# sbi-dev/sbi

Hardware: AMD Instinct MI355X
Metric: NPE train (theta,x)-pairs/sec (higher is better)
Workload: dtype f32; 1 GPU; BASELINE configs[1]: NPE + NSF theta-dim 10, x-dim 10, 100000 simulations (90 000-row training split resident in HBM), batch 65536 per GPU, synthetic linear-Gaussian; step = shuffled batch gather (device sampler) + fused NPE training step (pack, loss fwd+bwd, grad all-reduce, clip+Adam); parallelism=dp1, rccl_ranks=1

## Files before the change

sbi_amd/csrc/nsf_train_kernel.h:

```cpp
#pragma once
#include <hip/hip_runtime.h>
#include <stdlib.h>
#include <string.h>
#include "nsf_device.h"
#include "nsf_plan_layout.h"

#define TR_NW 4
#define TR_ROWS 64
#define TR_MAXCH 4
#define TR_GRID_MAX 256
#define TR_SA 68
#define TR_SB 68
#define TR_SLOT(PT) (16 * (PT) + 1)
#define TR_LDK_FAST 50
#ifndef TR_LA
#define TR_LA 2
#endif
#ifndef TR_SPLINE_PRIO
#define TR_SPLINE_PRIO 0
#endif
#ifndef TR_H_SPLIT
#define TR_H_SPLIT 0
#endif
#ifndef TR_PSTASH
#define TR_PSTASH 1
#endif
#ifndef TR_NO_S0
#define TR_NO_S0 1
#endif

struct TrainPlan {
  int SA, SB, SS;
  int o_A0, o_A1, o_B, o_Bs, o_cnt;
  int o_xs;
  int o_wave, w_total;
  int w_zs, w_gys, w_gzs;
  int DCHB, PTW;
  int nch[2];
  int PLP;
  int grid, ntiles;
  int lds_floats;
  int overlay;
  float* grad_x;
};

constexpr int build_train_layout(const NsfPlan& pl, TrainPlan* tp) {
  if (pl.D > 15 || pl.H > 64 || pl.NB > 2 || (pl.NB < 1 && !pl.ctx_mlp)) return SBI_AMD_E_UNSUPPORTED;
  const int d_id_max = pl.shape[0].d_id > pl.shape[1].d_id ? pl.shape[0].d_id : pl.shape[1].d_id;
  if (d_id_max + pl.C + 1 > 32 || pl.C + 1 > 32) return SBI_AMD_E_UNSUPPORTED;
  tp->DCHB = 4 / pl.PT;
  if (tp->DCHB < 1) return SBI_AMD_E_UNSUPPORTED;
  if (tp->DCHB > 2) tp->DCHB = 2;
  tp->PTW = 16 * pl.PT;
  for (int par = 0; par < 2; ++par) {
    tp->nch[par] = (pl.shape[par].d_tr + tp->DCHB - 1) / tp->DCHB;
    if (tp->nch[par] > TR_MAXCH) return SBI_AMD_E_UNSUPPORTED;
  }
  tp->SA = TR_SA;
  tp->SB = TR_SB;
  {
    const int in0max = d_id_max + pl.C;
    const int nt0 = (in0max + 1 + 15) / 16, ntc = (pl.C + 1 + 15) / 16;
    int need = 16 * nt0 > d_id_max + 16 * ntc ? 16 * nt0 : d_id_max + 16 * ntc;
    tp->SS = (need + 3) / 4 * 4;
    if ((tp->SS / 4) % 2 == 0) tp->SS += 4;
  }
  int w = 0;
  tp->w_zs = w; w += 16 * pl.ZW;
  tp->w_gys = w; w += 16 * pl.ZW;
  tp->w_gzs = w; w += 16 * pl.ZW;
  tp->w_total = (w + 16 + 3) / 4 * 4;
  for (int ov = 0; ov < 2; ++ov) {
    const int fin_min = pl.shape[0].final_off < pl.shape[1].final_off ? pl.shape[0].final_off : pl.shape[1].final_off;
    int o = ov ? (pl.hidden_img_floats > pl.lds_w_train_floats - fin_min ? pl.hidden_img_floats
                                                                         : pl.lds_w_train_floats - fin_min)
               : pl.lds_w_train_floats;
    o = (o + 3) / 4 * 4;
    tp->overlay = ov;
    tp->o_A0 = o; o += TR_ROWS * tp->SA;
    tp->o_A1 = o; o += TR_ROWS * tp->SA;
    tp->o_B = o; o += TR_ROWS * tp->SB;
    tp->o_Bs = o; o += TR_ROWS * tp->SS;
    tp->o_cnt = o; o += 4;
    tp->o_xs = o; o += 64;
    tp->o_wave = o;
    tp->lds_floats = tp->o_wave + TR_NW * tp->w_total;
    if (4ll * tp->lds_floats <= NSF_LDS_LIMIT_BYTES) break;
  }
  if (4ll * tp->lds_floats > NSF_LDS_LIMIT_BYTES) return SBI_AMD_E_LDS;
  int pmax = pl.shape[0].n_params > pl.shape[1].n_params ? pl.shape[0].n_params : pl.shape[1].n_params;
  tp->PLP = (pmax + 1 + 3) / 4 * 4;
  tp->grad_x = nullptr;
  tp->ntiles = 0;
  tp->grid = 0;
  return 0;
}
static int build_train_plan(const NsfPlan& pl, int64_t n, TrainPlan* tp) {
  *tp = TrainPlan{};
  const int rc = build_train_layout(pl, tp);
  if (rc) return rc;
  tp->ntiles = (int)((n + TR_ROWS - 1) / TR_ROWS);
  tp->grid = tp->ntiles < TR_GRID_MAX ? tp->ntiles : TR_GRID_MAX;
  if (NSF_DBG_ABL(pl.ablate, 512) && tp->grid > 4) tp->grid = 4;
  return 0;
}

constexpr sbi_amd_nsf_config kNsfDefaultCfg = {10, 10, 50, 10, 5, 2, 3.0f, 1e-3f, 1e-3f, 1e-3f, 1e-3f};
constexpr NsfPlan nsf_make_static_plan() {
  NsfPlan p{};
  nsf_build_layout(&kNsfDefaultCfg, TR_NW, &p);
  return p;
}
constexpr NsfPlan kStaticPl = nsf_make_static_plan();
constexpr TrainPlan nsf_make_static_train() {
  TrainPlan t{};
  build_train_layout(kStaticPl, &t);
  return t;
}
constexpr TrainPlan kStaticTp = nsf_make_static_train();
static_assert(kStaticPl.n_params == 98025 && kStaticTp.overlay == 0 && kStaticTp.nch[0] == 3, "default NSF layout");

static bool plan_is_static_default(const NsfPlan& pl, const TrainPlan& tp) {
  NsfPlan a = pl;
  a.B = a.min_w = a.min_h = a.min_d = a.lu_eps = a.sqrt_h = a.inv_sqrt_h = 0.f;
  a.one_minus_kw = a.one_minus_kh = a.d_const = a.log_z = 0.f;
  a.ablate = 0;
  const NsfPlan b = kStaticPl;
  if (memcmp(&a, &b, sizeof(NsfPlan)) != 0) return false;
  TrainPlan c = tp;
  c.grid = c.ntiles = 0;
  c.grad_x = nullptr;
  const TrainPlan d = kStaticTp;
  return memcmp(&c, &d, sizeof(TrainPlan)) == 0 && NSF_DBG_ABL(pl.ablate, 0x40000) == 0;
}

__device__ __forceinline__ void stage_D(float* __restrict__ st, int SA, int row, const LaneId& id,
                                        const f4 (&v)[NSF_HT], bool relu) {
#pragma unroll
  for (int mt = 0; mt < NSF_HT; ++mt)
#pragma unroll
    for (int r = 0; r < 4; ++r) {
      float a = v[mt][r];
      st[row * SA + 16 * mt + 4 * r + id.g] = relu ? fmaxf(a, 0.f) : a;
    }
}

__device__ __forceinline__ int il_col(int c) { return 4 * (c & 15) + (c >> 4); }
__device__ __forceinline__ void stage_DB(float* __restrict__ st, int SB, int row, const LaneId& id,
                                         const f4 (&v)[NSF_HT], bool relu) {
  static_assert(NSF_HT == 4, "one float4 per register row");
#pragma unroll
  for (int r = 0; r < 4; ++r) {
    f4 w = {v[0][r], v[1][r], v[2][r], v[3][r]};
    if (relu) w = {fmaxf(w[0], 0.f), fmaxf(w[1], 0.f), fmaxf(w[2], 0.f), fmaxf(w[3], 0.f)};
    *(f4*)(st + row * SB + 4 * (4 * r + id.g)) = w;
  }
}

__device__ __forceinline__ constexpr int dw_krow(int s) { return 16 * (s >> 2) + (s & 3); }

template <int NT, int SA, int SB, bool IL = false>
__device__ __forceinline__ void dw_gemm(const float* __restrict__ Ast, const float* __restrict__ Bst,
                                        int acol0, int bcol0, const LaneId& id, f4 (&acc)[NT], int nt_on = NT,
                                        int abl = 0, f4* accb = nullptr) {
  if (abl & 1) return;
  const float ones_b = id.j == 0 ? 1.f : 0.f;
  constexpr int KS = TR_ROWS / 4, LA = NT >= 3 ? TR_LA : 2 * TR_LA;
  const float* ap = Ast + 4 * id.g * SA + acol0 + id.j;
  const float* bp = IL ? Bst + 4 * id.g * SB + 4 * id.j + (bcol0 >> 4) : Bst + 4 * id.g * SB + bcol0 + id.j;
  float a[LA + 1], b[LA + 1][NT];
  auto load_b = [&](int u, int s) {
    if (IL && NT == 4) {
      const f4 w = *(const f4*)(bp + dw_krow(s) * SB);
#pragma unroll
      for (int nt = 0; nt < NT; ++nt) b[u][nt] = w[nt];
    } else {
#pragma unroll
      for (int nt = 0; nt < NT; ++nt) b[u][nt] = bp[dw_krow(s) * SB + (IL ? nt : 16 * nt)];
    }
  };
#pragma unroll
  for (int u = 0; u < LA; ++u) {
    a[u] = ap[dw_krow(u) * SA];
    load_b(u, u);
  }
#pragma unroll
  for (int s = 0; s < KS; ++s) {
    if (s + LA < KS) {
      a[(s + LA) % (LA + 1)] = ap[dw_krow(s + LA) * SA];
      load_b((s + LA) % (LA + 1), s + LA);
    }
    __builtin_amdgcn_sched_barrier(0);
#pragma unroll
    for (int nt = 0; nt < NT; ++nt)
      if (NT == 1 || nt < nt_on) acc[nt] = MFMA16(a[s % (LA + 1)], b[s % (LA + 1)][nt], acc[nt]);
    if (accb) *accb = MFMA16(a[s % (LA + 1)], ones_b, *accb);
    __builtin_amdgcn_sched_barrier(0);
  }
}

template <int NT, int SA>
__device__ __forceinline__ void dw_gemm_rs(const float* __restrict__ Ast, const float* __restrict__ Bst, int SBr,
                                           int acol0, int bcol0, const LaneId& id, f4 (&acc)[NT], int nt_on = NT,
                                           int abl = 0) {
  if (abl & 1) return;
  constexpr int KS = TR_ROWS / 4, LA = NT >= 4 ? TR_LA : 2 * TR_LA;
  const float* ap = Ast + 4 * id.g * SA + acol0 + id.j;
  const float* bp = Bst + 4 * id.g * SBr + bcol0 + id.j;
  float a[LA + 1], b[LA + 1][NT];
#pragma unroll
  for (int u = 0; u < LA; ++u) {
    a[u] = ap[dw_krow(u) * SA];
#pragma unroll
    for (int nt = 0; nt < NT; ++nt) b[u][nt] = bp[dw_krow(u) * SBr + 16 * nt];
  }
#pragma unroll
  for (int s = 0; s < KS; ++s) {
    if (s + LA < KS) {
      a[(s + LA) % (LA + 1)] = ap[dw_krow(s + LA) * SA];
#pragma unroll
      for (int nt = 0; nt < NT; ++nt) b[(s + LA) % (LA + 1)][nt] = bp[dw_krow(s + LA) * SBr + 16 * nt];
    }
    __builtin_amdgcn_sched_barrier(0);
#pragma unroll
    for (int nt = 0; nt < NT; ++nt)
      if (NT == 1 || nt < nt_on) acc[nt] = MFMA16(a[s % (LA + 1)], b[s % (LA + 1)][nt], acc[nt]);
    __builtin_amdgcn_sched_barrier(0);
  }
}

#define MFMA4(a, b, c) __builtin_amdgcn_mfma_f32_4x4x1f32((a), (b), (c), 0, 0, 0)
constexpr int TR_THIN_C0 = 48;
static_assert(kStaticPl.H == TR_THIN_C0 + 2 && kStaticPl.KSH == 13 && kStaticPl.NB == 2,
              "thin remainder: the static layout's hidden width leaves 2 real features (+ bias column) in tile 3");

template <int SA, int SB>
__device__ __forceinline__ void dw_thin(const float* __restrict__ Ast, const float* __restrict__ Bst, const LaneId& id,
                                        f4& accM, f4& accN) {
  const int l = id.lane;
  const float* aM = Ast + TR_THIN_C0 + (l & 3);
  const float* aN = Ast + l;
  const float* bM = Bst + il_col(l);
  const float* bN = Bst + il_col(TR_THIN_C0 + (l & 3));
  constexpr int KS = TR_ROWS / 4;
  float v[2][4][4];
  auto load = [&](int u, int s) {
#pragma unroll
    for (int g = 0; g < 4; ++g) {
      const int r = dw_krow(s) + 4 * g;
      v[u][g][0] = aM[r * SA];
      v[u][g][1] = bM[r * SB];
      v[u][g][2] = aN[r * SA];
      v[u][g][3] = bN[r * SB];
    }
  };
  load(0, 0);
#pragma unroll
  for (int s = 0; s < KS; ++s) {
    if (s + 1 < KS) load((s + 1) & 1, s + 1);
    __builtin_amdgcn_sched_barrier(0);
#pragma unroll
    for (int g = 0; g < 4; ++g) {
      accM = MFMA4(v[s & 1][g][0], v[s & 1][g][1], accM);
      accN = MFMA4(v[s & 1][g][2], v[s & 1][g][3], accN);
    }
    __builtin_amdgcn_sched_barrier(0);
  }
}
template <bool THIN>
__device__ __forceinline__ void dw_hidden(const float* __restrict__ Ast, const float* __restrict__ Bst, int gw,
                                          const LaneId& id, f4 (&acc)[4], int abl) {
  if constexpr (THIN) {
    if (abl & 1) return;
    if (gw == TR_NW - 1) dw_thin<TR_SA, TR_SB>(Ast, Bst, id, acc[0], acc[1]);
    else dw_gemm<3, TR_SA, TR_SB, true>(Ast, Bst, 16 * gw, 0, id, *reinterpret_cast<f4(*)[3]>(&acc[0]));
  } else {
    dw_gemm<4, TR_SA, TR_SB, true>(Ast, Bst, 16 * gw, 0, id, acc, 4, abl, nullptr);
  }
}

__device__ __forceinline__ void load_D(const float* __restrict__ st, int SA, int row, const LaneId& id,
                                       f4 (&v)[NSF_HT]) {
#pragma unroll
  for (int mt = 0; mt < NSF_HT; ++mt)
#pragma unroll
    for (int r = 0; r < 4; ++r) v[mt][r] = st[row * SA + 16 * mt + 4 * r + id.g];
}

__device__ __forceinline__ void grad_wave_sync(int* cnt, int target, int lane) {
  __builtin_amdgcn_fence(__ATOMIC_RELEASE, "workgroup");
  if (lane == 0) __hip_atomic_fetch_add(cnt, 1, __ATOMIC_RELAXED, __HIP_MEMORY_SCOPE_WORKGROUP);
  while (__hip_atomic_load(cnt, __ATOMIC_RELAXED, __HIP_MEMORY_SCOPE_WORKGROUP) < target) __builtin_amdgcn_s_sleep(1);
  __builtin_amdgcn_fence(__ATOMIC_ACQUIRE, "workgroup");
}

template <int KS, int MT, int LDK>
__device__ __forceinline__ void gemm_T_breg_ldk(const float* __restrict__ lds, const LinDesc& L, const LaneId& id,
                                                const f4 (&gb)[NSF_HT], f4 (&acc)[MT]) {
  const int ldk = LDK ? LDK : L.ldk;
  const float* base[MT];
#pragma unroll
  for (int mt = 0; mt < MT; ++mt) {
    const int f = 16 * mt + id.iperm;
    base[mt] = lds + L.l_w + id.g * ldk + (f < L.in ? f : 0);
  }
  const int kstride = 4 * ldk;
  constexpr int NP = (KS + 1) / 2;
  float a[2][2][MT];
#pragma unroll
  for (int u = 0; u < 2; ++u)
#pragma unroll
    for (int mt = 0; mt < MT; ++mt) a[0][u][mt] = u < KS ? base[mt][u * kstride] : 0.f;
#pragma unroll
  for (int p = 0; p < NP; ++p) {
    if (p + 1 < NP) {
#pragma unroll
      for (int u = 0; u < 2; ++u)
#pragma unroll
        for (int mt = 0; mt < MT; ++mt)
          a[(p + 1) & 1][u][mt] = (2 * p + 2 + u < KS) ? base[mt][(2 * p + 2 + u) * kstride] : 0.f;
    }
    __builtin_amdgcn_sched_barrier(0);
#pragma unroll
    for (int u = 0; u < 2; ++u) {
      const int s = 2 * p + u;
      if (s < KS) {
        const float bv = gb[s >> 2][s & 3];
#pragma unroll
        for (int mt = 0; mt < MT; ++mt) acc[mt] = MFMA16(a[p & 1][u][mt], bv, acc[mt]);
      }
    }
// ... 254 lines not shown
      }
    }
  }
#pragma unroll
  for (int mt = 0; mt < NSF_HT; ++mt)
#pragma unroll
    for (int r = 0; r < 4; ++r) gh[mt][r] = (16 * mt + 4 * r + id.g < LF.in) ? gh[mt][r] : 0.f;
}
template <int PT>
__device__ __forceinline__ void wft_chunk(const float* __restrict__ lds, const LinDesc& LF, const NsfPlan& pl,
                                          const ShapeDesc& S, const LaneId& id, const float* __restrict__ Arow,
                                          int SA, int d0, f4 (&gh)[NSF_HT]) {
  if (LF.ldk == TR_LDK_FAST) wft_chunk_ldk<PT, TR_LDK_FAST>(lds, LF, pl, S, id, Arow, SA, d0, gh);
  else wft_chunk_ldk<PT, 0>(lds, LF, pl, S, id, Arow, SA, d0, gh);
}

__device__ __forceinline__ void write_tile(float* __restrict__ part, const LinDesc& L, int out0, int nt,
                                           const LaneId& id, const f4& acc) {
#pragma unroll
  for (int r = 0; r < 4; ++r) {
    const int out = out0 + 4 * id.g + r;
    const int in = 16 * nt + id.j;
    if (out < L.out) {
      if (in < L.in) part[L.g_w + out * L.in + in] = acc[r];
      else if (in == L.in) part[L.g_b + out] = acc[r];
    }
  }
}
__device__ __forceinline__ void write_thin(float* __restrict__ part, const LinDesc& L, const LaneId& id, const f4& accM,
                                           const f4& accN) {
  const int l = id.lane;
#pragma unroll
  for (int m = 0; m < 4; ++m) {
    const int outM = TR_THIN_C0 + m, inM = l;
    if (outM < L.out) {
      if (inM < L.in) part[L.g_w + outM * L.in + inM] = accM[m];
      else if (inM == L.in) part[L.g_b + outM] = accM[m];
    }
    const int outN = 4 * (l >> 2) + m, inN = TR_THIN_C0 + (l & 3);
    if (l < TR_THIN_C0 && outN < L.out) {
      if (inN < L.in) part[L.g_w + outN * L.in + inN] = accN[m];
      else if (inN == L.in) part[L.g_b + outN] = accN[m];
    }
  }
}
__device__ __forceinline__ void write_bias(float* __restrict__ part, const LinDesc& L, int out0, const LaneId& id,
                                           const f4& accb) {
  if (id.j != 0) return;
#pragma unroll
  for (int r = 0; r < 4; ++r) {
    const int out = out0 + 4 * id.g + r;
    if (out < L.out) part[L.g_b + out] = accb[r];
  }
}

constexpr LinDesc wo_lin(int i) { return kStaticPl.shape[0].lin[i]; }
#define WO_LANE_WORDS(L, row0, in)                                    \
  const bool wcol_ = (in) < (L).in;                                   \
  const int off = wcol_ ? (L).g_w + ((row0) + 4 * g) * (L).in + (in) : (L).g_b + (row0) + 4 * g; \
  const int stride = wcol_ ? (L).in : 1;
template <int LI, int GW, int NT>
__device__ __forceinline__ void wo_tiles(float* __restrict__ part, int j, int g, const f4* acc) {
  constexpr LinDesc L = wo_lin(LI);
  constexpr int rem = L.out - 16 * GW;
  static_assert(rem >= 16 || (rem > 0 && rem <= 4), "a partial m-tile's live rows sit in lane group 0");
  constexpr int RL = rem >= 16 ? 4 : rem;
#pragma unroll
  for (int nt = 0; nt < NT; ++nt) {
    if (16 * nt > L.in) continue;
    const int in = 16 * nt + j;
    WO_LANE_WORDS(L, 16 * GW, in)
    bool live = in <= L.in;
    if (rem < 16) live = live && g == 0;
    if (live) {
#pragma unroll
      for (int r = 0; r < RL; ++r) part[off + r * stride] = acc[nt][r];
    }
  }
}
template <int LI>
__device__ __forceinline__ void wo_thin(float* __restrict__ part, int l, const f4& accM, const f4& accN) {
  constexpr LinDesc L = wo_lin(LI);
  static_assert(L.out == TR_THIN_C0 + 2 && L.in == L.out, "thin strips: a 50 x 50 hidden layer");
  if (l <= L.in) {
    const bool w = l < L.in;
    const int off = w ? L.g_w + TR_THIN_C0 * L.in + l : L.g_b + TR_THIN_C0;
    const int stride = w ? L.in : 1;
#pragma unroll
    for (int m = 0; m < L.out - TR_THIN_C0; ++m) part[off + m * stride] = accM[m];
  }
  const int in = TR_THIN_C0 + (l & 3);
  if (l < TR_THIN_C0 && in <= L.in) {
    const bool w = in < L.in;
    const int row = 4 * (l >> 2);
    const int off = w ? L.g_w + row * L.in + in : L.g_b + row;
    const int stride = w ? L.in : 1;
#pragma unroll
    for (int m = 0; m < 4; ++m) part[off + m * stride] = accN[m];
  }
}
template <int DD, int PTI, int NT0, int NTN>
__device__ __forceinline__ void wo_final(float* __restrict__ part, int j, int g, const f4* acc) {
  constexpr LinDesc L = wo_lin(kStaticPl.shape[0].fin);
  constexpr int P = kStaticPl.P;
  constexpr int rem = P - 16 * PTI;
  static_assert(rem > 0, "parameter tile");
  constexpr int GF = rem / 4, RP = rem % 4;
#pragma unroll
  for (int i = 0; i < NTN; ++i) {
    if (16 * (NT0 + i) > L.in) continue;
    const int in = 16 * (NT0 + i) + j;
    WO_LANE_WORDS(L, DD * P + 16 * PTI, in)
    const bool live = in <= L.in;
    if (live && g <= GF) {
#pragma unroll
      for (int r = 0; r < RP; ++r) part[off + r * stride] = acc[i][r];
    }
    if (live && g < GF) {
#pragma unroll
      for (int r = RP; r < 4; ++r) part[off + r * stride] = acc[i][r];
    }
  }
}
template <int GW>
__device__ __forceinline__ void wo_lu(float* __restrict__ part, int j, int g, const f4& acc) {
  constexpr int D = kStaticPl.D, ntri = D * (D - 1) / 2;
  constexpr int o_low = kStaticPl.shape[0].g_lu, o_up = o_low + ntri, o_diag = o_up + ntri, o_bias = o_diag + D;
#pragma unroll
  for (int r = 0; r < 4; ++r) {
    const int i = 4 * g + r, k = j;
    if (GW == 0) {
      const bool tri = i < D && k < D && k >= i, lad = i == D && k == D;
      const int off = lad ? kStaticPl.shape[0].n_params
                          : (k > i ? o_up + i * D - i * (i + 1) / 2 + (k - i - 1) : o_diag + i);
      if (tri || lad) part[off] = acc[r];
    } else {
      const bool low = i < D && k < i, bias = i < D && k == D;
      const int off = bias ? o_bias + i : o_low + i * (i - 1) / 2 + k;
      if (low || bias) part[off] = acc[r];
    }
  }
}
#undef WO_LANE_WORDS
template <int GW>
__device__ __forceinline__ void wo_static(float* __restrict__ part, int j, int g, int l, const f4 (&acc0)[1],
                                          const f4 (&accC)[2][1], const f4 (&acc1)[2][4], const f4 (&acc2)[2][4],
                                          const f4 (&accF)[3][4], const f4& accLU) {
  constexpr int PT = kStaticPl.PT, d_tr = kStaticPl.shape[0].d_tr;
  static_assert(kStaticPl.NB == 2 && PT == 2 && kStaticTp.nch[0] == 3 && (d_tr & 1) && d_tr == 5 && TR_NW == 4,
                "chunks of two dims, the last one split (see the chunk steps)");
  wo_tiles<0, GW, 1>(part, j, g, acc0);
  wo_tiles<1, GW, 1>(part, j, g, accC[0]);
  wo_tiles<4, GW, 1>(part, j, g, accC[1]);
  if constexpr (GW == TR_NW - 1) {
    wo_thin<2>(part, l, acc1[0][0], acc1[0][1]);
    wo_thin<3>(part, l, acc2[0][0], acc2[0][1]);
    wo_thin<5>(part, l, acc1[1][0], acc1[1][1]);
    wo_thin<6>(part, l, acc2[1][0], acc2[1][1]);
  } else {
    wo_tiles<2, GW, 3>(part, j, g, acc1[0]);
    wo_tiles<3, GW, 3>(part, j, g, acc2[0]);
    wo_tiles<5, GW, 3>(part, j, g, acc1[1]);
    wo_tiles<6, GW, 3>(part, j, g, acc2[1]);
  }
  wo_final<0 + GW / PT, GW % PT, 0, 4>(part, j, g, accF[0]);
  wo_final<2 + GW / PT, GW % PT, 0, 4>(part, j, g, accF[1]);
  wo_final<4, GW % PT, PT * (GW / PT), PT>(part, j, g, accF[2]);
  if constexpr (GW < 2) wo_lu<GW>(part, j, g, accLU);
}

__device__ __forceinline__ constexpr int cm_reps(const NsfPlan& pl) { return pl.ctx_reps; }
struct BwdIo {
  int t_hi, t_lo;
  const float* packed;
  const float* zstats;
  const float* stash;
  const float* x;
  const float* noise;
  float* gz[2];
  const float* row_w;
  float uni_w;
  long long n, x_rows;
  float* partial;
  float* grad_theta;
  const float* astash;
  const float* pstash;
  long long* dbg;
};
template <int K, int KSH, int NBT, int NCH, int NTW, bool HB, int SP = 0>
__global__ void __launch_bounds__(128 * TR_NW, HB ? 1 : 2)
nsf_bwd_layer_kernel(const NsfPlan pl_, const TrainPlan tp_, const BwdIo io) {
  const float* __restrict__ packed = io.packed;
  const float* __restrict__ zstats = io.zstats;
  const float* __restrict__ x = io.x;
  const float* __restrict__ row_w = io.row_w;
  const float uni_w = io.uni_w;
  const long long n = io.n, x_rows = io.x_rows;
  float* __restrict__ partial = io.partial;
  float* __restrict__ grad_theta = io.grad_theta;
  const float* __restrict__ astash = io.astash;
  long long* __restrict__ dbg = io.dbg;
  const NsfPlan& pl = SP != 0 ? kStaticPl : pl_;
  const TrainPlan& tp = SP != 0 ? kStaticTp : tp_;
#ifdef NSF_DEBUG
  const int dbg_tile_sel = pl_.ablate & 128;
#define NSF_ABL(bit) (pl_.ablate & (bit))
#define NSF_ABLV (pl_.ablate)
#define TS(i) do { if (dbg && t == 0 && blockIdx.x == 0 && (threadIdx.x & 63) == 0 && tile == (int)(blockIdx.x + (dbg_tile_sel ? gridDim.x : 0))) \
    dbg[(threadIdx.x >> 6) * 64 + (i)] = (long long)__builtin_readcyclecounter(); } while (0)
#define TSX(i) do { if (dbg && t < 8 && blockIdx.x == 0 && (threadIdx.x & 63) == 0) \
    dbg[512 + (threadIdx.x >> 6) * 64 + 8 * t + (i)] = (long long)__builtin_readcyclecounter(); } while (0)
#else
#define TSX(i) do { } while (0)
#define NSF_ABL(bit) 0
#define NSF_ABLV 0
#define TS(i) do { } while (0)
#endif
  constexpr int PT = (3 * K - 1 + 15) / 16;
  constexpr int DCHB = (4 / PT) > 2 ? 2 : (4 / PT);
  extern __shared__ __attribute__((aligned(16))) float lds[];
  const int tid = threadIdx.x;
  const int wave = tid >> 6;
  const LaneId id = make_lane();
  constexpr bool cm = (NBT == 0);
  constexpr int NB = cm ? 1 : NBT;
  const int SLOTS = nsf_ast_slots(pl);
  const int reps = cm_reps(pl);
  const int D = pl.D, C = pl.C;
  constexpr int SA = TR_SA, SB = TR_SB;
  const int SS = tp.SS;
  float* Bt = lds + tp.o_B;
  float* Bs = lds + tp.o_Bs;
  const float* x_mean = zstats + 2 * D;
  const float* x_std = x_mean + C;

  if (NSF_ABL(256)) {
    for (int i = tid; i < tp.lds_floats; i += blockDim.x) lds[i] = __builtin_nanf("");
    __syncthreads();
  }
  const bool ov = tp.overlay != 0;
  if (!ov) stage_layer(lds, packed + (long long)io.t_hi * pl.img_floats, pl.lds_w_train_floats, tid, blockDim.x);
  if (tid == 0) *(int*)(lds + tp.o_cnt) = 0;
  if (tid < 32) {
    lds[tp.o_xs + tid] = tid < C ? x_mean[tid] : 0.f;
    lds[tp.o_xs + 32 + tid] = tid < C ? 1.f / x_std[tid] : 1.f;
  }
  const float* xs = lds + tp.o_xs;
  const int ntc = (C + 1 + 15) / 16;
  const f4 zero4 = {0.f, 0.f, 0.f, 0.f};
  const bool multi = (int)(blockIdx.x + gridDim.x) < tp_.ntiles;
#define BWD_T_VARS                                                                                                  \
  const int par = cm ? 0 : (t & 1);                                                                                 \
  const ShapeDesc& S = pl.shape[(SP != 0 || cm) ? 0 : par];                                                         \
  const bool is_last = (t == pl.T - 1);                                                                             \
  const float* img = packed + (long long)t * pl.img_floats;                                                         \
  const int F0 = ov ? S.final_off : 0;                                                                              \
  const float* ldsF = lds - F0;                                                                                     \
  const LinDesc& L0 = S.lin[0];                                                                                     \
  const LinDesc& LF = S.lin[S.fin];                                                                                 \
  const int nch = tp.nch[(SP != 0 || cm) ? 0 : par];                                                                \
  const int nt0 = (S.in0 + 1 + 15) / 16;                               \
                     \
  const int o_AX = (nch & 1) ? tp.o_A1 : tp.o_A0;                                                                   \
  const int o_AY = (nch & 1) ? tp.o_A0 : tp.o_A1;                                                                   \
  (void)img; (void)L0; (void)LF; (void)nt0; (void)o_AX; (void)o_AY; (void)ldsF; (void)is_last;

  if (wave < TR_NW) {
    float* sc = lds + tp.o_wave + wave * tp.w_total;
    float* zs = sc + tp.w_zs;
    float* gys = sc + tp.w_gys;
    float* gzs = sc + tp.w_gzs;
    const int arow0 = 16 * wave;
    for (int i = id.lane; i < tp.w_total; i += 64) sc[i] = 0.f;
    const int bs_live = (pl.shape[0].in0 > pl.shape[1].in0 ? pl.shape[0].in0 : pl.shape[1].in0) + 1;
    for (int i = id.lane; i < 16 * SS; i += 64) Bs[arow0 * SS + i] = 0.f;
    const LaneId id0 = id;
    float zv[4], gv[4], xv[8], wv;
    auto fetch_inputs = [&](int t_, int tile_, const LaneId& id) {
      const long long row_ = (long long)tile_ * TR_ROWS + arow0 + id.j;
      const long long rs = row_ < n ? row_ : 0;
      const long long xr = (x_rows == n) ? rs : (x_rows == 1 ? 0 : rs % x_rows);
      const float* z_in = io.stash + (long long)t_ * n * D;
      const float* gz_up = (t_ == pl.T - 1) ? io.noise : io.gz[(t_ + 1) & 1];
      const int d_id_ = pl.shape[(SP != 0 || cm) ? 0 : (t_ & 1)].d_id;
#pragma unroll
      for (int u = 0; u < 4; ++u) {
        const int d = id.g + 4 * u;
        const int dc = d < D ? d : 0;
        zv[u] = z_in[rs * D + dc];
        gv[u] = __hip_atomic_load(gz_up + rs * D + dc, __ATOMIC_RELAXED, __HIP_MEMORY_SCOPE_AGENT);
      }
#pragma unroll
      for (int u = 0; u < 8; ++u) {
        const int c = id.g + 4 * u - d_id_;
        xv[u] = x[xr * C + ((c >= 0 && c < C) ? c : 0)];
      }
      wv = row_w ? row_w[rs] : uni_w;
    };
    for (int t = io.t_hi; t >= io.t_lo; --t) {
    BWD_T_VARS
    LaneId id = id0;
    asm volatile("" : "+v"(id.lane), "+v"(id.j), "+v"(id.g), "+v"(id.iperm));
    float* __restrict__ gz_dn = io.gz[t & 1];
    if (t == io.t_hi || !multi) fetch_inputs(t, blockIdx.x, id);
    for (int tile = blockIdx.x; tile < tp_.ntiles; tile += gridDim.x) {
      LaneId id = id0;
      asm volatile("" : "+v"(id.j), "+v"(id.g), "+v"(id.iperm));
      const long long row = (long long)tile * TR_ROWS + arow0 + id.j;
      const bool valid = row < n;
      const float wn = valid ? wv : 0.f;
      const float gld = -wn;
      const int trow = arow0 + id.j;
      const bool need_s0 = !TR_NO_S0 || ov || tile == (int)blockIdx.x;
      if (need_s0) { TSX(4); __syncthreads(); TSX(5); }
      if (ov) {
        stage_layer(lds, img + F0, pl.lds_w_train_floats - F0, tid, blockDim.x);
        __syncthreads();
      }
      TS(0);
      float gzr[4];
      {
#pragma unroll
        for (int u = 0; u < 4; ++u) {
          const int d = id.g + 4 * u;
          const float gz = (valid && d < D) ? gv[u] : 0.f;
          gzr[u] = is_last ? wn * gz : gz;
          if (d < D) {
            zs[id.j * pl.ZW + d] = valid ? zv[u] : 0.f;
            gzs[id.j * pl.ZW + d] = gzr[u];
          }
        }
        wave_lds_fence();
#pragma unroll
        for (int u = 0; u < 8; ++u) {
          if (4 * u >= bs_live) break;
          const int k = id.g + 4 * u;
          const int c = k - S.d_id;
          const int cc = (c >= 0 && c < C) ? c : 0;
          const int zd = 2 * k + (1 - par);
          const float zid = zs[id.j * pl.ZW + (zd < D ? zd : 0)];
          const float ctx = ((valid ? xv[u] : 0.f) - xs[cc]) * xs[32 + cc];
          float v = (k == S.in0) ? 1.f : 0.f;
          v = (c >= 0 && c < C) ? ctx : v;
          v = (k < S.d_id) ? zid : v;
          if (k < SS) Bs[trow * SS + k] = v;
        }
      }
      float gus_r[4] = {0.f, 0.f, 0.f, 0.f};
      if (cm) {
        for (int k = id.g; k < D; k += 4) gys[id.j * pl.ZW + k] = gzs[id.j * pl.ZW + k];
      } else if (!(NSF_ABL(64))) {
        const float* Lm = ldsF + S.l_L;
        const float* Um = ldsF + S.l_U;
        f4 gu = zero4, gy = zero4;
        float al[4], bz[4], au[4];
#pragma unroll
        for (int s4 = 0; s4 < 4; ++s4) {
          al[s4] = Lm[(4 * s4 + id.g) * 16 + id.j];
          bz[s4] = gzr[s4];
          au[s4] = Um[(4 * id.g + s4) * 16 + id.j];
        }
#pragma unroll
        for (int s4 = 0; s4 < 4; ++s4) gu = MFMA16(al[s4], bz[s4], gu);
#pragma unroll
        for (int s4 = 0; s4 < 4; ++s4) gy = MFMA16(au[s4], gu[s4], gy);
#pragma unroll
        for (int ii = 0; ii < 4; ++ii) {
          gus_r[ii] = gu[ii];
          if (4 * id.g + ii < D) gys[id.j * pl.ZW + 4 * id.g + ii] = gy[ii];
        }
      }
      wave_lds_fence();
      const long long nt16 = (n + 15) / 16;
      const long long wt16 = (long long)tile * TR_NW + wave < nt16 ? (long long)tile * TR_NW + wave : nt16 - 1;
      const float* ast = astash + (((long long)t * nt16 + wt16) * SLOTS) * 1024 +
                         4 * id.lane;
      TS(1);
      __syncthreads();
      TS(2);

      f4 bt1[NSF_HT], bt2[NSF_HT], bsg[NSF_HT];
      f4 hpre[cm ? 2 : 1][NSF_HT];
      if (TR_SPLINE_PRIO) __builtin_amdgcn_s_setprio(TR_SPLINE_PRIO);
      for (int c = 0; c < nch; ++c) {
        const int d0 = c * DCHB;
        const int slot = id.g & 1, part = id.g >> 1;
        const int dd = d0 + slot;
        float* pp = lds + ((c & 1) ? tp.o_A1 : tp.o_A0) + trow * SA + slot * TR_SLOT(PT);
        if (slot < DCHB) {
          if (dd < S.d_tr && !(NSF_ABL(4))) {
            const int zi = id.j * pl.ZW + 2 * dd + par;
            float yv, gxv;
            rq_spline_pair_bwd<K>(pp, tp.PTW, zs[zi], gys[zi], gld, pl_, part, yv, gxv);
            if (part == 0) {
              zs[zi] = yv;
              gys[zi] = gxv;
            }
          } else if (part == 0) {
            for (int k = 0; k < tp.PTW; ++k) pp[k] = 0.f;
          }
        }
        TS(3 + c);
        __syncthreads();
      }
      if (TR_SPLINE_PRIO) __builtin_amdgcn_s_setprio(0);
      if (cm) {
        ast_load<KSH>(ast, reps > 0 ? reps - 1 : 0, hpre[0]);
        if (reps > 0) ast_load<KSH>(ast, reps, hpre[1]);
      } else {
        ast_load<KSH>(ast, 2 + 4 * (NB - 1), bt2);
        ast_load<KSH>(ast, 3 + 4 * (NB - 1), bsg);
        ast_load<KSH>(ast, 1 + 4 * (NB - 1), bt1);
      }
      float us_r[4] = {0.f, 0.f, 0.f, 0.f};
      if (!cm && !(NSF_ABL(64))) {
        const float* Um = ldsF + S.l_U;
        float au[4], by[4];
#pragma unroll
        for (int s4 = 0; s4 < 4; ++s4) {
          au[s4] = Um[id.j * 16 + 4 * s4 + id.g];
          by[s4] = zs[id.j * pl.ZW + 4 * s4 + id.g];
        }
        f4 uv = zero4;
#pragma unroll
        for (int s4 = 0; s4 < 4; ++s4) uv = MFMA16(au[s4], by[s4], uv);
#pragma unroll
        for (int ii = 0; ii < 4; ++ii) us_r[ii] = uv[ii];
      }
      {
        const int nxt = tile + (int)gridDim.x;
        const bool more = nxt < tp_.ntiles, hop = !more && multi && t > io.t_lo;
        fetch_inputs(hop ? t - 1 : t, more ? nxt : (hop ? (int)blockIdx.x : tile), id);
      }
      TS(8);
      __syncthreads();
      if (ov) {
        stage_layer(lds, img, S.final_off, tid, blockDim.x);
        __syncthreads();
      }
      TS(9);
      const bool hsplit = TR_H_SPLIT && !cm && !ov;
      f4 gh[NSF_HT];
      load_D(lds + o_AX, SA, trow, id, gh);
      wave_lds_fence();
      const bool want_gx = tp_.grad_x != nullptr;
      float* gx_row = want_gx ? tp_.grad_x + (valid ? row : 0) * C : nullptr;

      if (cm) {
        f4 ga[NSF_HT], gb[NSF_HT];
        for (int i = reps; i >= 1; --i) {
          if (i < reps) {
            ast_load<KSH>(ast, i - 1, hpre[0]);
            ast_load<KSH>(ast, i, hpre[1]);
            __syncthreads();
          }
#pragma unroll
          for (int mt = 0; mt < NSF_HT; ++mt)
#pragma unroll
            for (int r = 0; r < 4; ++r) ga[mt][r] = hpre[1][mt][r] > 0.f ? gh[mt][r] : 0.f;
          stage_D(lds + o_AY, SA, trow, id, ga, false);
          stage_DB(Bt, SB, trow, id, hpre[0], true);
          if (!HB && id.g == 0) Bt[trow * SB + il_col(pl.H)] = 1.f;
          __syncthreads();
#pragma unroll
          for (int mt = 0; mt < NSF_HT; ++mt) gb[mt] = zero4;
          gemm_T_breg<KSH, NSF_HT>(lds, S.lin[1], id, ga, gb, NSF_ABLV);
#pragma unroll
          for (int mt = 0; mt < NSF_HT; ++mt) gh[mt] = gb[mt];
        }
#pragma unroll
        for (int mt = 0; mt < NSF_HT; ++mt)
#pragma unroll
          for (int r = 0; r < 4; ++r) gh[mt][r] = hpre[0][mt][r] > 0.f ? gh[mt][r] : 0.f;
      } else {
#pragma unroll
        for (int b = NB - 1; b >= 0; --b) {
          f4 ga[NSF_HT], gb[NSF_HT];
          {
            f4 gc[NSF_HT];
#pragma unroll
            for (int mt = 0; mt < NSF_HT; ++mt)
#pragma unroll
              for (int r = 0; r < 4; ++r) {
                const float sgm = bsg[mt][r];
                ga[mt][r] = gh[mt][r] * sgm;
                gc[mt][r] = gh[mt][r] * bt2[mt][r] * sgm * (1.f - sgm);
              }
            stage_D(lds + o_AX, SA, trow, id, gc, false);
            if (want_gx)
              ctx_grad_update<KSH>(lds, S.lin[1 + 3 * b], id, gc, 0, C, xs, gx_row, valid, is_last && b == NB - 1);
            if (hsplit && b == NB - 1) {
              TS(50);
              __syncthreads();
              TS(51);
            }
            stage_D(lds + o_AY, SA, trow, id, ga, false);
          }
          stage_DB(Bt, SB, trow, id, bt1, true);
          if (!HB && id.g == 0) Bt[trow * SB + il_col(pl.H)] = 1.f;
          ast_load<KSH>(ast, 4 * b, hpre[0]);
          if (b > 0) {
            ast_load<KSH>(ast, 2 + 4 * (b - 1), bt2);
            ast_load<KSH>(ast, 3 + 4 * (b - 1), bsg);
          }
          TS(20 + 8 * b);
          __syncthreads();
          TS(21 + 8 * b);
#pragma unroll
          for (int mt = 0; mt < NSF_HT; ++mt) gb[mt] = zero4;
          gemm_T_breg<KSH, NSF_HT>(lds, S.lin[3 + 3 * b], id, ga, gb, NSF_ABLV);
#pragma unroll
          for (int mt = 0; mt < NSF_HT; ++mt)
#pragma unroll
            for (int r = 0; r < 4; ++r) ga[mt][r] = bt1[mt][r] > 0.f ? gb[mt][r] : 0.f;
          if (b > 0) ast_load<KSH>(ast, 1 + 4 * (b - 1), bt1);
          TS(22 + 8 * b);
          __syncthreads();
          TS(23 + 8 * b);
          stage_D(lds + o_AY, SA, trow, id, ga, false);
          stage_DB(Bt, SB, trow, id, hpre[0], true);
          if (!HB && id.g == 0) Bt[trow * SB + il_col(pl.H)] = 1.f;
          __syncthreads();
          TS(24 + 8 * b);
#pragma unroll
          for (int mt = 0; mt < NSF_HT; ++mt) gb[mt] = zero4;
          gemm_T_breg<KSH, NSF_HT>(lds, S.lin[2 + 3 * b], id, ga, gb, NSF_ABLV);
#pragma unroll
          for (int mt = 0; mt < NSF_HT; ++mt)
#pragma unroll
            for (int r = 0; r < 4; ++r) gh[mt][r] += hpre[0][mt][r] > 0.f ? gb[mt][r] : 0.f;
          TS(25 + 8 * b);
          if (b > 0) __syncthreads();
        }
      }

      stage_D(lds + o_AX, SA, trow, id, gh, false);
      TS(40);
      __syncthreads();
      TS(41);
      {
        f4 gin[1];
        gin[0] = zero4;
        gemm_T_breg<KSH, 1>(lds, L0, id, gh, gin, NSF_ABLV);
#pragma unroll
        for (int r = 0; r < 4; ++r) {
          const int k = 4 * r + id.g;
          if (k < S.d_id) gys[id.j * pl.ZW + 2 * k + (1 - par)] += gin[0][r];
        }
      }
      if (want_gx) ctx_grad_update<KSH>(lds, L0, id, gh, S.d_id, C, xs, gx_row, valid, is_last && cm);
      if (!cm) {
        float* Ay = lds + o_AY + trow * SA;
#pragma unroll
        for (int ii = 0; ii < 4; ++ii) {
          const int k = 4 * id.g + ii;
          const int o = id.j * pl.ZW + k;
          Ay[k] = k < D ? gus_r[ii] : (k == D ? gld : 0.f);
          Ay[16 + k] = k < D ? gzs[o] : 0.f;
          Bt[trow * SB + il_col(k)] = k < D ? zs[o] : (k == D ? 1.f : 0.f);
          Bt[trow * SB + il_col(16 + k)] = k < D ? us_r[ii] : (k == D ? 1.f : 0.f);
        }
      }
      TS(42);
      __syncthreads();
      for (int d = id.g; d < D; d += 4) {
        if (valid) {
          const float g = gys[id.j * pl.ZW + d];
          if (t > 0) gz_dn[row * D + d] = g;
          else if (grad_theta) grad_theta[row * D + d] = g * zstats[D + d];
        }
      }
      TS(43);
    }
    TSX(2);
    if (t > io.t_lo && !ov) stage_layer(lds, packed + (long long)(t - 1) * pl.img_floats, pl.lds_w_train_floats, tid, 64 * TR_NW);
    TSX(3);
    }

  } else {
    const int gw = wave - TR_NW;
    int* cnt = (int*)(lds + tp.o_cnt);
    int sync_target = 0;
    const LaneId id0 = id;
    f4 hl[NSF_HT];
    auto fetch_hl = [&](int t_, int tile_) {
      const long long nt16 = (n + 15) / 16;
      const long long wt16 = (long long)tile_ * TR_NW + gw < nt16 ? (long long)tile_ * TR_NW + gw : nt16 - 1;
      const float* ast = astash + (((long long)t_ * nt16 + wt16) * SLOTS) * 1024 +
                         4 * id0.lane;
      ast_load<KSH>(ast, cm ? reps : 4 * NB, hl);
    };
    constexpr bool use_pst = TR_PSTASH != 0;
    f4 pq[DCHB][PT];
    auto pq_load = [&](int t_, int tile_, int c_) {
      const long long nt16 = (n + 15) / 16;
      const long long wt16 = (long long)tile_ * TR_NW + gw < nt16 ? (long long)tile_ * TR_NW + gw : nt16 - 1;
      const float* pstw = io.pstash + ((long long)t_ * nt16 + wt16) * nsf_pst_tile_floats(pl) + 4 * id0.lane;
      const int d_tr_ = pl.shape[(SP != 0 || cm) ? 0 : (t_ & 1)].d_tr;
#pragma unroll
      for (int sl = 0; sl < DCHB; ++sl) {
        const int dd = c_ * DCHB + sl;
#pragma unroll
        for (int pt = 0; pt < PT; ++pt) pq[sl][pt] = pst_load<PT>(pstw, dd < d_tr_ ? dd : d_tr_ - 1, pt);
      }
    };
    auto pq_store = [&](float* __restrict__ arow, const LaneId& id, int c_, int d_tr_) {
#pragma unroll
      for (int sl = 0; sl < DCHB; ++sl)
        if (c_ * DCHB + sl < d_tr_) {
#pragma unroll
          for (int pt = 0; pt < PT; ++pt)
#pragma unroll
            for (int r = 0; r < 4; ++r) arow[id.j * SA + sl * TR_SLOT(PT) + 16 * pt + 4 * r + id.g] = pq[sl][pt][r];
        }
    };
    fetch_hl(io.t_hi, blockIdx.x);
    if (use_pst) pq_load(io.t_hi, blockIdx.x, 0);
    for (int t = io.t_hi; t >= io.t_lo; --t) {
    BWD_T_VARS
    LaneId id = id0;
    asm volatile("" : "+v"(id.lane), "+v"(id.j), "+v"(id.g), "+v"(id.iperm));
    f4 acc0[NTW], accC[NB][NTW], acc1[NB][4], acc2[NB][4], accF[NCH][4], accLU[1];
    f4 acc1b[HB ? NB : 1], acc2b[HB ? NB : 1], accFb[HB ? NCH : 1];
  #pragma unroll
    for (int i = 0; i < (HB ? NB : 1); ++i) { acc1b[i] = zero4; acc2b[i] = zero4; }
  #pragma unroll
    for (int i = 0; i < (HB ? NCH : 1); ++i) accFb[i] = zero4;
  #pragma unroll
    for (int i = 0; i < NTW; ++i) acc0[i] = zero4;
  #pragma unroll
    for (int b = 0; b < NB; ++b) {
  #pragma unroll
      for (int i = 0; i < NTW; ++i) accC[b][i] = zero4;
  #pragma unroll
      for (int i = 0; i < 4; ++i) { acc1[b][i] = zero4; acc2[b][i] = zero4; }
    }
  #pragma unroll
    for (int c = 0; c < NCH; ++c)
  #pragma unroll
      for (int i = 0; i < 4; ++i) accF[c][i] = zero4;
    accLU[0] = zero4;

    for (int tile = blockIdx.x; tile < tp_.ntiles; tile += gridDim.x) {
      LaneId id = id0;
      asm volatile("" : "+v"(id.j), "+v"(id.g), "+v"(id.iperm));
      const int trow = 16 * gw + id.j;
      const bool more_tiles = tile + (int)gridDim.x < tp_.ntiles;
      const int t_nxt = more_tiles ? t : (t > io.t_lo ? t - 1 : t);
      const int tile_nxt = more_tiles ? tile + (int)gridDim.x : (t > io.t_lo ? (int)blockIdx.x : tile);
      const bool need_s0 = !TR_NO_S0 || ov || tile == (int)blockIdx.x;
      if (need_s0) { TSX(4); __syncthreads(); TSX(5); }
      else { sync_target += 4; grad_wave_sync(cnt, sync_target, id.lane); }
      if (ov) {
        stage_layer(lds, img + F0, pl.lds_w_train_floats - F0, tid, blockDim.x);
        __syncthreads();
      }
      TS(0);
      stage_DB(Bt, SB, trow, id, hl, false);
      if (!HB && id.g == 0) Bt[trow * SB + il_col(pl.H)] = 1.f;
      if (use_pst) {
        pq_store(lds + tp.o_A0 + 16 * gw * SA, id, 0, S.d_tr);
        if (1 < nch) pq_load(t, tile, 1);
      } else if (!(NSF_ABL(32))) final_layer_chunk_T<PT, KSH>(ldsF, lds + tp.o_A0 + 16 * gw * SA, pl, tp, S, id, hl, 0);
      f4 gh[NSF_HT];
  #pragma unroll
      for (int mt = 0; mt < NSF_HT; ++mt) gh[mt] = zero4;
      TS(1);
      __syncthreads();
      TS(2);
  #pragma unroll
      for (int k = 0; k <= NCH; ++k) {
        if (k <= nch) {
          if (k >= 1) {
            const int oa = ((k - 1) & 1) ? tp.o_A1 : tp.o_A0;
            const bool hsplit = TR_H_SPLIT && !cm && !ov;
            if (hsplit && k == nch) {
              if (!(NSF_ABL(2))) wft_chunk<PT>(ldsF, LF, pl, S, id, lds + oa + 16 * gw * SA, SA, (k - 1) * DCHB, gh);
              stage_D(lds + o_AX, SA, trow, id, gh, false);
              TS(9);
              __syncthreads();
            }
            if (!HB && DCHB == 2 && k == nch && (S.d_tr & 1)) {
              f4 (&af)[4] = accF[k - 1 < NCH ? k - 1 : 0];
              f4 part[PT < 3 ? PT : 1];
#pragma unroll
              for (int i = 0; i < (PT < 3 ? PT : 1); ++i) part[i] = af[i];
              dw_gemm<(PT < 3 ? PT : 1), TR_SA, TR_SB, true>(lds + oa, Bt, 16 * (gw % PT), 16 * PT * (gw / PT), id, part,
                                                             PT < 3 ? PT : 1, NSF_ABLV, nullptr);
#pragma unroll
              for (int i = 0; i < (PT < 3 ? PT : 1); ++i) af[i] = part[i];
            } else
            dw_gemm<4, TR_SA, TR_SB, true>(lds + oa, Bt, 16 * gw + (gw / PT < DCHB ? gw / PT : 0), 0, id,
                                           accF[k - 1 < NCH ? k - 1 : 0], 4, NSF_ABLV,
                                           HB ? &accFb[k - 1 < NCH ? k - 1 : 0] : nullptr);
            TS(13 + k);
            if (!(hsplit && k == nch) && !(NSF_ABL(2)))
              wft_chunk<PT>(ldsF, LF, pl, S, id, lds + oa + 16 * gw * SA, SA, (k - 1) * DCHB, gh);
          }
          TS(3 + 2 * k);
          if (k + 1 < nch) {
            if (k >= 1) { sync_target += 4; grad_wave_sync(cnt, sync_target, id.lane); }
            TS(17 + k);
            if (use_pst) {
              pq_store(lds + (((k + 1) & 1) ? tp.o_A1 : tp.o_A0) + 16 * gw * SA, id, k + 1, S.d_tr);
              if (k + 2 < nch) pq_load(t, tile, k + 2);
            } else if (!(NSF_ABL(32)))
              final_layer_chunk_T<PT, KSH>(ldsF, lds + (((k + 1) & 1) ? tp.o_A1 : tp.o_A0) + 16 * gw * SA, pl, tp, S, id,
                                           hl, (k + 1) * DCHB);
          }
          if (k == nch && !(TR_H_SPLIT && !cm && !ov)) stage_D(lds + o_AX, SA, trow, id, gh, false);
          TS(4 + 2 * k);
          __syncthreads();
          if (ov && k == nch) {
            stage_layer(lds, img, S.final_off, tid, blockDim.x);
            __syncthreads();
          }
        }
      }
      if (cm) {
        for (int i = reps; i >= 1; --i) {
          if (i < reps) __syncthreads();
          __syncthreads();
          dw_gemm<4, TR_SA, TR_SB, true>(lds + o_AY, Bt, 16 * gw, 0, id, acc1[0], 4, NSF_ABLV, HB ? &acc1b[0] : nullptr);
        }
      } else {
  #pragma unroll
        for (int b = NB - 1; b >= 0; --b) {
          __syncthreads();
          TS(21 + 8 * b);
          if constexpr (SP != 0) dw_hidden<true>(lds + o_AY, Bt, gw, id, acc2[b], NSF_ABLV);
          else dw_gemm<4, TR_SA, TR_SB, true>(lds + o_AY, Bt, 16 * gw, 0, id, acc2[b], 4, NSF_ABLV, HB ? &acc2b[b] : nullptr);
          TS(22 + 8 * b);
          __syncthreads();
          dw_gemm_rs<NTW, TR_SA>(lds + o_AX, Bs, SS, 16 * gw, S.d_id, id, accC[b], ntc, NSF_ABLV);
          __syncthreads();
          TS(24 + 8 * b);
          if constexpr (SP != 0) dw_hidden<true>(lds + o_AY, Bt, gw, id, acc1[b], NSF_ABLV);
          else dw_gemm<4, TR_SA, TR_SB, true>(lds + o_AY, Bt, 16 * gw, 0, id, acc1[b], 4, NSF_ABLV, HB ? &acc1b[b] : nullptr);
          TS(25 + 8 * b);
          if (b > 0) __syncthreads();
        }
      }
      __syncthreads();
      TS(41);
      fetch_hl(t_nxt, tile_nxt);
      if (use_pst) pq_load(t_nxt, tile_nxt, 0);
      dw_gemm_rs<NTW, TR_SA>(lds + o_AX, Bs, SS, 16 * gw, 0, id, acc0, nt0, NSF_ABLV);
      TS(42);
      __syncthreads();
      if (gw < 2 && !cm) dw_gemm<1, TR_SA, TR_SB, true>(lds + o_AY, Bt, 16 * gw, 16 * gw, id, accLU);
      TS(43);
    }

    TSX(0);
    float* part = partial + ((long long)t * gridDim.x + blockIdx.x) * tp.PLP;
    if constexpr (SP != 0) {
      const int j = id.j & 15, g = id.g & 3, l = id.lane & 63;
      switch (__builtin_amdgcn_readfirstlane(gw)) {
        case 0: wo_static<0>(part, j, g, l, acc0, accC, acc1, acc2, accF, accLU[0]); break;
        case 1: wo_static<1>(part, j, g, l, acc0, accC, acc1, acc2, accF, accLU[0]); break;
        case 2: wo_static<2>(part, j, g, l, acc0, accC, acc1, acc2, accF, accLU[0]); break;
        default: wo_static<3>(part, j, g, l, acc0, accC, acc1, acc2, accF, accLU[0]); break;
      }
    } else {
    const int out0 = 16 * gw;
  #pragma unroll
    for (int nt = 0; nt < NTW; ++nt) write_tile(part, L0, out0, nt, id, acc0[nt]);
    if (cm) {
  #pragma unroll
      for (int nt = 0; nt < 4; ++nt) write_tile(part, S.lin[1], out0, nt, id, acc1[0][nt]);
      if (HB) write_bias(part, S.lin[1], out0, id, acc1b[0]);
    } else {
  #pragma unroll
      for (int b = 0; b < NB; ++b) {
  #pragma unroll
        for (int nt = 0; nt < NTW; ++nt) write_tile(part, S.lin[1 + 3 * b], out0, nt, id, accC[b][nt]);
        if (SP != 0 && gw == TR_NW - 1) {
          write_thin(part, S.lin[2 + 3 * b], id, acc1[b][0], acc1[b][1]);
          write_thin(part, S.lin[3 + 3 * b], id, acc2[b][0], acc2[b][1]);
        } else {
  #pragma unroll
          for (int nt = 0; nt < (SP != 0 ? 3 : 4); ++nt) {
            write_tile(part, S.lin[2 + 3 * b], out0, nt, id, acc1[b][nt]);
            write_tile(part, S.lin[3 + 3 * b], out0, nt, id, acc2[b][nt]);
          }
        }
        if (HB) {
          write_bias(part, S.lin[2 + 3 * b], out0, id, acc1b[b]);
          write_bias(part, S.lin[3 + 3 * b], out0, id, acc2b[b]);
        }
      }
    }
  #pragma unroll
    for (int c = 0; c < NCH; ++c) {
      if (c < nch) {
        if (!HB && DCHB == 2 && c == nch - 1 && (S.d_tr & 1)) {
          const int dd = c * DCHB, pt = gw % PT;
  #pragma unroll
          for (int i = 0; i < (PT < 3 ? PT : 1); ++i)
  #pragma unroll
            for (int r = 0; r < 4; ++r) {
              const int p = 16 * pt + 4 * id.g + r;
              const int in = 16 * (PT * (gw / PT) + i) + id.j;
              if (p < pl.P) {
                const int out = dd * pl.P + p;
                if (in < LF.in) part[LF.g_w + out * LF.in + in] = accF[c][i][r];
                else if (in == LF.in) part[LF.g_b + out] = accF[c][i][r];
              }
            }
          continue;
        }
        const int dd = c * DCHB + gw / PT;
        const int pt = gw % PT;
        if (gw < DCHB * PT && dd < S.d_tr) {
  #pragma unroll
          for (int nt = 0; nt < 4; ++nt)
  #pragma unroll
            for (int r = 0; r < 4; ++r) {
              const int p = 16 * pt + 4 * id.g + r;
              const int in = 16 * nt + id.j;
              if (p < pl.P) {
                const int out = dd * pl.P + p;
                if (in < LF.in) part[LF.g_w + out * LF.in + in] = accF[c][nt][r];
                else if (in == LF.in) part[LF.g_b + out] = accF[c][nt][r];
                if (HB && nt == 0 && id.j == 0) part[LF.g_b + out] = accFb[c][r];
              }
            }
        }
      }
    }
    if (!cm) {
      const int ntri = D * (D - 1) / 2;
      float* plow = part + S.g_lu;
      float* pup = plow + ntri;
      float* pdiag = pup + ntri;
      float* pbias = pdiag + D;
  #pragma unroll
      for (int r = 0; r < 4; ++r) {
        const int i = 4 * id.g + r, k = id.j;
        const float v = accLU[0][r];
        if (gw == 0) {
          if (i < D && k < D) {
            if (k > i) pup[i * D - i * (i + 1) / 2 + (k - i - 1)] = v;
            else if (k == i) pdiag[i] = v;
          } else if (i == D && k == D) part[S.n_params] = v;
        } else if (gw == 1) {
          if (i < D) {
            if (k < i) plow[i * (i - 1) / 2 + k] = v;
            else if (k == D) pbias[i] = v;
          }
        }
      }
    }
    }
    TSX(1);
    }

  }
#undef BWD_T_VARS
#undef NSF_ABL
#undef NSF_ABLV
#undef TS
#undef TSX
}


template <int K, int KSH, int NB, int NCH, int NTW, bool HB = false, int SP = 0>
static int launch_bwd(const NsfPlan& pl, const TrainPlan& tp, const BwdIo& io, hipStream_t st) {
  auto kern = nsf_bwd_layer_kernel<K, KSH, NB, NCH, NTW, HB, SP>;
  const int lds_bytes = 4 * tp.lds_floats;
  hipError_t e = hipFuncSetAttribute((const void*)kern, hipFuncAttributeMaxDynamicSharedMemorySize, lds_bytes);
  if (e != hipSuccess) return (int)e;
  hipLaunchKernelGGL(kern, dim3(tp.grid), dim3(128 * TR_NW), (size_t)lds_bytes, st, pl, tp, io);
  return (int)hipGetLastError();
}

template <int K>
static int launch_bwd_one(const NsfPlan& pl, const TrainPlan& tp, const BwdIo& io, int nchmax, bool wide, hipStream_t st) {
// ... 62 lines not shown
```

Before: 96.03 million pairs/s.

## Hoist loop-invariant LU/context loads and skip dead gradient work in NSF backward

Hoists the per-layer LU-matrix and context-normalisation LDS loads out of the per-tile loop so they are read once per layer pass. Reorders the first LU MFMA ahead of the z/gz LDS stores to overlap them, and splits the context packing into a load phase and a compute phase. Skips the input-gradient GEMM and global writes at the first layer when grad_theta is not requested, and skips zeroing dead spline parameter slots. This adds register pressure from the hoisted arrays and relies on those LDS values staying fixed across tiles.

```diff
diff --git a/sbi_amd/csrc/nsf_train_kernel.h b/sbi_amd/csrc/nsf_train_kernel.h
--- a/sbi_amd/csrc/nsf_train_kernel.h
+++ b/sbi_amd/csrc/nsf_train_kernel.h
@@ -27,6 +27,12 @@
 #endif
 #ifndef TR_NO_S0
 #define TR_NO_S0 1
+#endif
+#ifndef TR_HOIST
+#define TR_HOIST 1
+#endif
+#ifndef TR_SKIP_DEAD
+#define TR_SKIP_DEAD 1
 #endif
 
 struct TrainPlan {
@@ -887,10 +893,25 @@
     LaneId id = id0;
     asm volatile("" : "+v"(id.lane), "+v"(id.j), "+v"(id.g), "+v"(id.iperm));
     float* __restrict__ gz_dn = io.gz[t & 1];
+    const bool need_gin = !TR_SKIP_DEAD || t > 0 || grad_theta != nullptr;
     if (t == io.t_hi || !multi) fetch_inputs(t, blockIdx.x, id);
+    constexpr int hoist = SP != 0 ? TR_HOIST : 0;
+    float al[4], au[4], uu[4], xm[8], xi[8];
+    const auto load_al = [&](const LaneId& id) {
+#pragma unroll
+      for (int s4 = 0; s4 < 4; ++s4) al[s4] = (ldsF + S.l_L)[(4 * s4 + id.g) * 16 + id.j];
+    };
+    const auto load_au = [&](const LaneId& id) {
+#pragma unroll
+      for (int s4 = 0; s4 < 4; ++s4) au[s4] = (ldsF + S.l_U)[(4 * id.g + s4) * 16 + id.j];
+    };
+    const auto load_uu = [&](const LaneId& id) {
+#pragma unroll
+      for (int s4 = 0; s4 < 4; ++s4) uu[s4] = (ldsF + S.l_U)[id.j * 16 + 4 * s4 + id.g];
+    };
     for (int tile = blockIdx.x; tile < tp_.ntiles; tile += gridDim.x) {
       LaneId id = id0;
-      asm volatile("" : "+v"(id.j), "+v"(id.g), "+v"(id.iperm));
+      asm volatile("" : "+v"(id.lane), "+v"(id.j), "+v"(id.g), "+v"(id.iperm));
       const long long row = (long long)tile * TR_ROWS + arow0 + id.j;
       const bool valid = row < n;
       const float wn = valid ? wv : 0.f;
@@ -903,19 +924,79 @@
         __syncthreads();
       }
       TS(0);
+      if (hoist >= 1 && tile == (int)blockIdx.x) {
+        if (!cm) {
+          load_al(id);
+          load_au(id);
+          if (hoist >= 2) load_uu(id);
+        }
+        if (hoist >= 3) {
+#pragma unroll
+          for (int u = 0; u < 8; ++u) {
+            if (4 * u >= bs_live) break;
+            const int c = id.g + 4 * u - S.d_id;
+            const int cc = (c >= 0 && c < C) ? c : 0;
+            xm[u] = xs[cc];
+            xi[u] = xs[32 + cc];
+          }
+        }
+      }
       float gzr[4];
-      {
-#pragma unroll
-        for (int u = 0; u < 4; ++u) {
-          const int d = id.g + 4 * u;
-          const float gz = (valid && d < D) ? gv[u] : 0.f;
-          gzr[u] = is_last ? wn * gz : gz;
-          if (d < D) {
-            zs[id.j * pl.ZW + d] = valid ? zv[u] : 0.f;
-            gzs[id.j * pl.ZW + d] = gzr[u];
+#pragma unroll
+      for (int u = 0; u < 4; ++u) {
+        const int d = id.g + 4 * u;
+        const float gz = (valid && d < D) ? gv[u] : 0.f;
+        gzr[u] = is_last ? wn * gz : gz;
+      }
+      const bool lu_mfma = !cm && !(NSF_ABL(64));
+      f4 gu = zero4, gy = zero4;
+      if (lu_mfma) {
+        if (hoist < 1) load_al(id);
+#pragma unroll
+        for (int s4 = 0; s4 < 4; ++s4) gu = MFMA16(al[s4], gzr[s4], gu);
+        if (hoist < 1) load_au(id);
+        asm volatile("" : "+v"(gu) : : "memory");
+      }
+#pragma unroll
+      for (int u = 0; u < 4; ++u) {
+        const int d = id.g + 4 * u;
+        if (d < D) {
+          zs[id.j * pl.ZW + d] = valid ? zv[u] : 0.f;
+          gzs[id.j * pl.ZW + d] = gzr[u];
+        }
+      }
+      wave_lds_fence();
+      if (lu_mfma) {
+#pragma unroll
+        for (int s4 = 0; s4 < 4; ++s4) gy = MFMA16(au[s4], gu[s4], gy);
+      }
+      if constexpr (SP != 0) {
+        float zid[8];
+#pragma unroll
+        for (int u = 0; u < 8; ++u) {
+          if (4 * u >= bs_live) break;
+          const int k = id.g + 4 * u;
+          const int c = k - S.d_id;
+          const int cc = (c >= 0 && c < C) ? c : 0;
+          const int zd = 2 * k + (1 - par);
+          zid[u] = 4 * u < S.d_id ? zs[id.j * pl.ZW + (zd < D ? zd : 0)] : 0.f;
+          if (hoist < 3) {
+            xm[u] = xs[cc];
+            xi[u] = xs[32 + cc];
           }
         }
-        wave_lds_fence();
+#pragma unroll
+        for (int u = 0; u < 8; ++u) {
+          if (4 * u >= bs_live) break;
+          const int k = id.g + 4 * u;
+          const int c = k - S.d_id;
+          const float ctx = ((valid ? xv[u] : 0.f) - xm[u]) * xi[u];
+          float v = (k == S.in0) ? 1.f : 0.f;
+          v = (c >= 0 && c < C) ? ctx : v;
+          v = (k < S.d_id) ? zid[u] : v;
+          if (4 * u + 3 < SS || k < SS) Bs[trow * SS + k] = v;
+        }
+      } else {
 #pragma unroll
         for (int u = 0; u < 8; ++u) {
           if (4 * u >= bs_live) break;
@@ -934,28 +1015,13 @@
       float gus_r[4] = {0.f, 0.f, 0.f, 0.f};
       if (cm) {
         for (int k = id.g; k < D; k += 4) gys[id.j * pl.ZW + k] = gzs[id.j * pl.ZW + k];
-      } else if (!(NSF_ABL(64))) {
-        const float* Lm = ldsF + S.l_L;
-        const float* Um = ldsF + S.l_U;
-        f4 gu = zero4, gy = zero4;
-        float al[4], bz[4], au[4];
-#pragma unroll
-        for (int s4 = 0; s4 < 4; ++s4) {
-          al[s4] = Lm[(4 * s4 + id.g) * 16 + id.j];
-          bz[s4] = gzr[s4];
-          au[s4] = Um[(4 * id.g + s4) * 16 + id.j];
-        }
-#pragma unroll
-        for (int s4 = 0; s4 < 4; ++s4) gu = MFMA16(al[s4], bz[s4], gu);
-#pragma unroll
-        for (int s4 = 0; s4 < 4; ++s4) gy = MFMA16(au[s4], gu[s4], gy);
+      } else if (lu_mfma) {
 #pragma unroll
         for (int ii = 0; ii < 4; ++ii) {
           gus_r[ii] = gu[ii];
           if (4 * id.g + ii < D) gys[id.j * pl.ZW + 4 * id.g + ii] = gy[ii];
         }
       }
-      wave_lds_fence();
       const long long nt16 = (n + 15) / 16;
       const long long wt16 = (long long)tile * TR_NW + wave < nt16 ? (long long)tile * TR_NW + wave : nt16 - 1;
       const float* ast = astash + (((long long)t * nt16 + wt16) * SLOTS) * 1024 +
@@ -981,7 +1047,7 @@
               zs[zi] = yv;
               gys[zi] = gxv;
             }
-          } else if (part == 0) {
+          } else if (part == 0 && !(TR_SKIP_DEAD && SP != 0 && dd >= S.d_tr)) {
             for (int k = 0; k < tp.PTW; ++k) pp[k] = 0.f;
           }
         }
@@ -999,16 +1065,15 @@
       }
       float us_r[4] = {0.f, 0.f, 0.f, 0.f};
       if (!cm && !(NSF_ABL(64))) {
-        const float* Um = ldsF + S.l_U;
-        float au[4], by[4];
+        float by[4];
 #pragma unroll
         for (int s4 = 0; s4 < 4; ++s4) {
-          au[s4] = Um[id.j * 16 + 4 * s4 + id.g];
           by[s4] = zs[id.j * pl.ZW + 4 * s4 + id.g];
         }
+        if (hoist < 2) load_uu(id);
         f4 uv = zero4;
 #pragma unroll
-        for (int s4 = 0; s4 < 4; ++s4) uv = MFMA16(au[s4], by[s4], uv);
+        for (int s4 = 0; s4 < 4; ++s4) uv = MFMA16(uu[s4], by[s4], uv);
 #pragma unroll
         for (int ii = 0; ii < 4; ++ii) us_r[ii] = uv[ii];
       }
@@ -1123,7 +1188,7 @@
       TS(40);
       __syncthreads();
       TS(41);
-      {
+      if (need_gin) {
         f4 gin[1];
         gin[0] = zero4;
         gemm_T_breg<KSH, 1>(lds, L0, id, gh, gin, NSF_ABLV);
@@ -1148,17 +1213,21 @@
       }
       TS(42);
       __syncthreads();
-      for (int d = id.g; d < D; d += 4) {
-        if (valid) {
-          const float g = gys[id.j * pl.ZW + d];
-          if (t > 0) gz_dn[row * D + d] = g;
-          else if (grad_theta) grad_theta[row * D + d] = g * zstats[D + d];
+      if (need_gin) {
+        for (int d = id.g; d < D; d += 4) {
+          if (valid) {
+            const float g = gys[id.j * pl.ZW + d];
+            if (t > 0) gz_dn[row * D + d] = g;
+            else if (grad_theta) grad_theta[row * D + d] = g * zstats[D + d];
+          }
         }
       }
       TS(43);
     }
     TSX(2);
-    if (t > io.t_lo && !ov) stage_layer(lds, packed + (long long)(t - 1) * pl.img_floats, pl.lds_w_train_floats, tid, 64 * TR_NW);
+    int tid_s = tid;
+    asm volatile("" : "+v"(tid_s));
+    if (t > io.t_lo && !ov) stage_layer(lds, packed + (long long)(t - 1) * pl.img_floats, pl.lds_w_train_floats, tid_s, 64 * TR_NW);
     TSX(3);
     }
 
```

Result: no change. 96.81 million pairs/s (median of 6 runs) (+0.8%).
